# bitfrozen/rendering-algorithms-raytracer

Measured on AMD Instinct MI355X. Metric: Mray/s (primary+shadow) on Sponza 1920x1080, higher is better.
Workload: dtype f32; 1 GPU; sponza stand-in (~66k tris) 1920x1080 Blinn+PointLight; config=C3, width=1920, height=1080, spp=1, qbvh_nodes=9084, qbvh_leaves=18162, frames_in_flight=4, hw_queues=4, parallelism=single GPU, whole frame

## Files before the change

### rendering-algorithms-raytracer_amd/csrc/mrt_frame.hip

```cpp
#include "mrt_kernels.h"
#include "mrt_shader.h"

namespace mrt {

template <bool COUNT, bool FAST, bool POW, int WALK = 1>
__device__ __forceinline__ v3 shade1_hit(const RenderParams& P, const Trav& T, TravStats& st, const DRay& r, float ht,
                                         float ha, float hb, int prim, const uint16_t* rcpT, const uint16_t* rsqT,
                                         uint32_t& shadow_total) {
    const v3 rayD = mk(r.d[0], r.d[1], r.d[2]);
    const PrimShade ps = P.prims[prim];
    const uint32_t mi = ps.mat;
    const bool lambert = P.mats[mi].type == MRT_LAMBERT;
    const float4 A = P.verts[ps.v[0]], B = P.verts[ps.v[1]], C = P.verts[ps.v[2]];
    const v3 geoN = normalized(cross(mk(B.x - A.x, B.y - A.y, B.z - A.z), mk(C.x - A.x, C.y - A.y, C.z - A.z)), rsqT);
    const float c = 1.0f - ha - hb;
    const float4 n0 = P.normals[ps.n[0]], n1 = P.normals[ps.n[1]], n2 = P.normals[ps.n[2]];
    const v3 N = normalized(add(add(scale(mk(n0.x, n0.y, n0.z), c), scale(mk(n1.x, n1.y, n1.z), ha)),
                                scale(mk(n2.x, n2.y, n2.z), hb)), rsqT);
    const v3 from = mk(r.o[0] + ht * r.d[0], r.o[1] + ht * r.d[1], r.o[2] + ht * r.d[2]);
    v3 n = N, rVec = mk(0, 0, 0);
    if (!lambert) {
        const v3 viewDir = neg(rayD);
        float vDotN = dot(viewDir, N);
        const float vDotGeoN = dot(viewDir, geoN);
        const bool same = (vDotN * vDotGeoN) >= 0.0f;
        n = same ? N : geoN;
        vDotN = same ? vDotN : vDotGeoN;
        if (vDotN < 0.0f) { vDotN = -vDotN; n = neg(n); }
        rVec = add(rayD, scale(n, 2.0f * vDotN));
    }
    const DevLight& l = P.lights[0];
    v3 L = sub(mk(l.pos[0], l.pos[1], l.pos[2]), from);
    float nDotL = dot(n, L);
    float e = 0.f, spec = 0.f;
    if (nDotL > 0.0f) {
        float falloff = dot(L, L);
        const float distanceRecip = rsqrt_nr(falloff, rsqT);
        falloff = rcp_nr(falloff, rcpT);
        const float distance = rcp_nr(distanceRecip, rcpT);
        L = scale(L, distanceRecip);
        nDotL *= distanceRecip;
        float Aterm = (l.power * falloff) * (0.25f / 3.1415926f);
        float rdl = std_max(0.f, dot(rVec, L));
        asm volatile("" : "+v"(Aterm), "+v"(rdl), "+v"(nDotL));
        float attenuate = 1.0f;
        if (l.cast_shadows) {
            const DRay sr = make_ray(from, L);
            DHit sh{distance, 0.f, 0.f, -1};
            shadow_total++;
            if (traverse<true, COUNT, FAST, false, true, WALK == 2, WALK != 0>(T, sr, 0.001f, sh, st)) attenuate = 0.0f;
        }
        attenuate *= nDotL;
        spec = rdl * attenuate;
        e = Aterm * attenuate;
    }
    const DevMaterial& M = P.mats[mi];
    const v3 E = mk(e, e, e);
    const v3 kd = mk(M.kd[0], M.kd[1], M.kd[2]), ka = mk(M.ka[0], M.ka[1], M.ka[2]);
    v3 sh;
    if (lambert) {
        sh = add(add(mk(0, 0, 0), mul(E, kd)), ka);
    } else {
        const v3 ks = mk(M.ks[0], M.ks[1], M.ks[2]);
        const float pw = (!POW || M.spec_exp == 1.0f) ? spec : spec_pow(spec, M.spec_exp);
        const v3 Ls = add(mk(0, 0, 0), scale(scale(mul(E, ks), M.spec_amt), pw));
        const v3 Ld = add(add(mk(0, 0, 0), mul(E, kd)), ka);
        const v3 z = mk(0, 0, 0);
        sh = add(add(scale(add(add(Ld, Ls), z), 1.0f), scale(add(z, z), 1.0f)), mk(M.le[0], M.le[1], M.le[2]));
    }
    return add(mk(0, 0, 0), sh);
}

template <bool COUNT, bool FAST, int MINW, bool POW>
__global__ void __launch_bounds__(kWG, MINW) shade1_kernel(RenderParams P) {
    __shared__ uint16_t s_tab[2048];
    __shared__ int32_t s_stack[kLdsStack * kWG];
    load_tables(P.tables, s_tab, 1024);
    const uint64_t t0 = (COUNT || P.wave_log) ? wall_clock64() : 0;
    const uint16_t* rcpT = s_tab;
    const uint16_t* rsqT = P.tables + 2048;
    const int tid = threadIdx.x, lane = tid & 63, wave = tid >> 6;
    Trav T{P.nodes, P.fast_box != 0, P.scalar_nodes, P.leaves, rcpT, s_stack + tid, P.gstack + (blockIdx.x * kWG + tid), P.gstride};
    T.inst = P.insts;
    trav_alpha(T, P);
    TravStats st;
    uint32_t shadow_total = 0;
    TileSched ts(P, wave, lane);
    uint32_t ntiles = 0;
    for (int item = ts.first(); item >= 0; item = ts.next(item)) {
        if (P.wave_log && lane == 0 && ntiles < kLogTiles)
        {
            unsigned long long* r = P.wave_log + kLogWords * ((size_t)blockIdx.x * (kWG / 64) + wave);
            r[4 + ntiles] = ((unsigned long long)item << 40) | (wall_clock64() & ((1ull << 40) - 1));
            r[4 + kLogTiles + ntiles] = ts.deq_ticks;
        }
        ntiles++;
        int x, y;
        size_t slot;
        if (!item_pixel(P, item, lane, x, y, slot)) continue;
        const float4 hv = P.hits[slot];
        const int prim = __float_as_int(hv.w);
        v3 col = mk(P.bg[0], P.bg[1], P.bg[2]);
        if (prim >= 0) {
            const int f = item_frame(P, item);
            const EyeRay er = camera_ray(P.cam[f], P.seed + (uint32_t)f, x, y, rsqT);
            col = shade1_hit<COUNT, FAST, POW>(P, T, st, make_ray(er.o, er.d), hv.x, hv.y, hv.z, prim, rcpT, rsqT, shadow_total);
        }
        item_pixel(P, item, lane, x, y, slot);
        store_rgb(P, slot, col);
    }
    flush_stats<COUNT, false>(P, st, shadow_total, lane, t0, ntiles);
}

template <bool COUNT, bool FAST, int MINW, bool POW, int WALK = 1>
__global__ void __launch_bounds__(kWG, MINW) frame1_kernel(RenderParams P) {
    constexpr bool LN = WALK == 2;
    __shared__ uint16_t s_tab[2048];
    __shared__ int32_t s_stack[kLdsStack * kWG];
    __shared__ QNode s_top[LN ? kLdsNodes : 1];
    if (LN)
        for (int i = threadIdx.x; i < kLdsNodes * 32; i += kWG)
            reinterpret_cast<uint32_t*>(s_top)[i] = reinterpret_cast<const uint32_t*>(P.nodes)[i];
    load_tables(P.tables, s_tab, 1024);
    const uint64_t t0 = (COUNT || P.wave_log) ? wall_clock64() : 0;
    const uint16_t* rcpT = s_tab;
    const uint16_t* rsqT = P.tables + 2048;
    const int tid = threadIdx.x, lane = tid & 63, wave = __builtin_amdgcn_readfirstlane(tid >> 6);
    Trav T{P.nodes, P.fast_box != 0, P.scalar_nodes, P.leaves, rcpT, s_stack + tid, P.gstack + (blockIdx.x * kWG + tid), P.gstride};
    T.inst = P.insts;
    trav_alpha(T, P);
    if (LN) T.lnodes = s_top;
    TravStats st, ss;
    uint32_t nhits = 0, shadow_total = 0;
    unsigned long long wave_steps = 0, wave_steps_s = 0;
    TileSched ts(P, wave, lane);
    uint32_t ntiles = 0;
    for (int item = ts.first(); item >= 0; item = ts.next(item)) {
        const RenderParams& PA = reload_params();
        if (PA.wave_log && lane_id() == 0 && ntiles < kLogTiles) {
            unsigned long long* r = PA.wave_log + kLogWords * ((size_t)blockIdx.x * (kWG / 64) + wave);
            r[4 + ntiles] = ((unsigned long long)item << 40) | (wall_clock64() & ((1ull << 40) - 1));
            r[4 + kLogTiles + ntiles] = ts.deq_ticks;
        }
        ntiles++;
        int x, y;
        size_t slot;
        const uint32_t n0 = st.nodes, s0 = ss.nodes;
        if (item_pixel(PA, item, lane_id(), x, y, slot)) {
            const int f = item_frame(PA, item);
            const EyeRay er = camera_ray(PA.cam[f], PA.seed + (uint32_t)f, x, y, rsqT);
            const DRay r = make_ray(er.o, er.d);
            DHit h{1e12f, 0.f, 0.f, -1};
            const bool hit = traverse<false, COUNT, FAST, false, true, LN, WALK != 0, WALK == 3>(T, r, 0.001f, h, st);
            const RenderParams& PB = reload_params();
            v3 col = mk(PB.bg[0], PB.bg[1], PB.bg[2]);
            if (hit) {
                nhits++;
                col = shade1_hit<COUNT, FAST, POW, WALK>(PB, T, ss, r, h.t, h.a, h.b, h.prim, rcpT, rsqT, shadow_total);
            }
            const RenderParams& PC = reload_params();
            item_pixel(PC, item, lane_id(), x, y, slot);
            if (PC.hits) PC.hits[slot] = make_float4(h.t, h.a, h.b, __int_as_float(hit ? h.prim : -1));
            store_rgb(PC, slot, col);
        }
        if (COUNT) {
            uint32_t dmax = st.nodes - n0, smax = ss.nodes - s0;
            for (int off = 32; off > 0; off >>= 1) {
                dmax = max(dmax, (uint32_t)__shfl_xor(dmax, off));
                smax = max(smax, (uint32_t)__shfl_xor(smax, off));
            }
            wave_steps += dmax;
            wave_steps_s += smax;
        }
    }
    if (COUNT) {
        unsigned long long sv = ss.nodes;
        for (int off = 32; off > 0; off >>= 1) sv += __shfl_down(sv, off);
        if (lane_id() == 0) {
            atomicAdd(&P.ctr[CTR_WAVE_STEPS_P], wave_steps);
            atomicAdd(&P.ctr[CTR_WAVE_STEPS_S], wave_steps_s);
            atomicAdd(&P.ctr[CTR_NODES_S], sv);
        }
    }
    flush_stats<COUNT, true>(P, st, nhits, lane_id(), t0, ntiles, ss.nodes, wave);
    flush_stats<COUNT, false, false>(P, ss, shadow_total, lane_id(), t0, ntiles, 0, wave);
}

template <int W, bool POW>
static KernelFn shade1_fn(bool c, bool f) {
    return c ? (f ? shade1_kernel<true, true, W, POW> : shade1_kernel<true, false, W, POW>)
             : (f ? shade1_kernel<false, true, W, POW> : shade1_kernel<false, false, W, POW>);
}
template <int W, bool POW, int WALK>
static KernelFn frame1_fn(bool c, bool f) {
    return c ? (f ? frame1_kernel<true, true, W, POW, WALK> : frame1_kernel<true, false, W, POW, WALK>)
             : (f ? frame1_kernel<false, true, W, POW, WALK> : frame1_kernel<false, false, W, POW, WALK>);
}
template <int WALK>
static KernelFn pick_frame1_walk(int w, bool c, bool f, bool pow) {
    if (pow) return w == 1 ? frame1_fn<1, true, WALK>(c, f) : frame1_fn<6, true, WALK>(c, f);
    switch (w) {
        case 1: return frame1_fn<1, false, WALK>(c, f);
        case 5: return frame1_fn<5, false, WALK>(c, f);
        case 7: return frame1_fn<7, false, WALK>(c, f);
        case 8: return frame1_fn<8, false, WALK>(c, f);
        default: return frame1_fn<6, false, WALK>(c, f);
    }
}
KernelFn pick_frame1(int w, bool c, bool f, bool pow, int walk) {
    switch (walk) {
        case 0: return pick_frame1_walk<0>(w, c, f, pow);
        case 2: return pick_frame1_walk<2>(w, c, f, pow);
        case 3: return pick_frame1_walk<3>(w, c, f, pow);
        default: return pick_frame1_walk<1>(w, c, f, pow);
    }
}
KernelFn pick_shade1(bool c, bool f, bool pow) { return pow ? shade1_fn<5, true>(c, f) : shade1_fn<5, false>(c, f); }
}
```

### rendering-algorithms-raytracer_amd/csrc/mrt_kernels.h

```cpp
#pragma once
#include <hip/hip_runtime.h>

#include "../../include/mrt.h"
#include "mrt_math.h"
#include "mrt_texture.h"
#include "mrt_types.h"

namespace mrt {

static constexpr int kWG = 256;
static constexpr int kLdsStack = 16;
static constexpr int kGlobalStack = 240;
static constexpr int kTableWords = 4096;
static constexpr int kLdsNodes = 64;

struct DRay {
    float o[3], d[3], id[3];
    bool finite;
    float time;
};

__device__ __forceinline__ DRay make_ray(v3 o, v3 d) {
    DRay r;
    r.o[0] = o.x; r.o[1] = o.y; r.o[2] = o.z;
    r.d[0] = d.x; r.d[1] = d.y; r.d[2] = d.z;
#pragma unroll
    for (int k = 0; k < 3; k++) {
        float v = 1.0f / r.d[k];
        if (r.d[k] == 0.f) v = (v < -0.f) ? -1e12f : 1e12f;
        r.id[k] = v;
    }
    r.finite = __builtin_isfinite(r.o[0]) & __builtin_isfinite(r.o[1]) & __builtin_isfinite(r.o[2]) &
               __builtin_isfinite(r.id[0]) & __builtin_isfinite(r.id[1]) & __builtin_isfinite(r.id[2]);
    r.time = 0.f;
    return r;
}
__device__ __forceinline__ DRay make_ray(v3 o, v3 d, float time) {
    DRay r = make_ray(o, d);
    r.time = time;
    return r;
}

struct DHit {
    float t, a, b;
    int32_t prim;
    int32_t inst = -1;
};

struct Trav {
    const QNode* __restrict__ nodes;
    bool fast_box;
    int scalar_nodes;
    const DLeaf* __restrict__ leaves;
    const uint16_t* rcpT;
    int32_t* lds;
    int32_t* gstk;
    uint32_t gstride;
    const DevInstance* inst = nullptr;
    const PrimShade* aprims = nullptr;
    const uint4* apuv = nullptr;
    const float2* auv = nullptr;
    const DevMaterial* amats = nullptr;
    const DevTexture* atex = nullptr;
    const uint8_t* pflags = nullptr;
    const float4* verts = nullptr;
    const float4* verts2 = nullptr;
    bool near_first = false;
    const QNode* lnodes = nullptr;
};

struct TravStats {
    uint32_t nodes = 0, leaves = 0, uniform = 0;
    int max_sp = 0;
    bool overflow = false;
};

__device__ __forceinline__ bool stk_push(const Trav& c, int& sp, int32_t v) {
    if (sp < kLdsStack) c.lds[sp * kWG] = v;
    else if (sp < kLdsStack + kGlobalStack) c.gstk[(size_t)(sp - kLdsStack) * c.gstride] = v;
    else return false;
    sp++;
    return true;
}
__device__ __forceinline__ int32_t stk_pop(const Trav& c, int& sp) {
    --sp;
    return sp < kLdsStack ? c.lds[sp * kWG] : c.gstk[(size_t)(sp - kLdsStack) * c.gstride];
}

__device__ __forceinline__ int32_t sel4(const int4& v, int i) {
    const int32_t lo = (i & 1) ? v.y : v.x, hi = (i & 1) ? v.w : v.z;
    return (i & 2) ? hi : lo;
}

__device__ __forceinline__ bool tri_test(const float* __restrict__ T, const DRay& r, float tMin, float tBest,
                                         float& ot, float& oa, float& ob, const uint16_t* rcpT) {
    const float ax = T[0], ay = T[1], az = T[2], e0x = T[3], e0y = T[4], e0z = T[5], e1x = T[6], e1y = T[7], e1z = T[8];
    const float px = r.d[1] * e1z - r.d[2] * e1y;
    const float py = -1.0f * (r.d[0] * e1z - r.d[2] * e1x);
    const float pz = r.d[0] * e1y - r.d[1] * e1x;
    const float det = e0x * px + (e0y * py + e0z * pz);
    const float inv = rcp_nr(det, rcpT);
    const float tx = r.o[0] - ax, ty = r.o[1] - ay, tz = r.o[2] - az;
    const float a = inv * (tx * px + (ty * py + tz * pz));
    if (__ballot((a >= 0.0f) & (a <= 1.0f)) == 0) {
        ot = a; oa = a; ob = a;
        return false;
    }
    const float qx = ty * e0z - tz * e0y;
    const float qy = -1.0f * (tx * e0z - tz * e0x);
    const float qz = tx * e0y - ty * e0x;
    const float b = inv * (r.d[0] * qx + (r.d[1] * qy + r.d[2] * qz));
    const float t = inv * (e1x * qx + (e1y * qy + e1z * qz));
    ot = t; oa = a; ob = b;
    return (a >= 0.0f) & (b >= 0.0f) & ((a + b) <= 1.0f) & (t >= tMin) & (t < tBest);
}

__device__ __forceinline__ int box_test(const float4* bx, const DRay& r, float tMin, float tMax) {
    float4 mnx = bx[0], mny = bx[1], mnz = bx[2], mxx = bx[3], mxy = bx[4], mxz = bx[5];
    float lx[4] = {mnx.x, mnx.y, mnx.z, mnx.w}, ly[4] = {mny.x, mny.y, mny.z, mny.w}, lz[4] = {mnz.x, mnz.y, mnz.z, mnz.w};
    float hx[4] = {mxx.x, mxx.y, mxx.z, mxx.w}, hy[4] = {mxy.x, mxy.y, mxy.z, mxy.w}, hz[4] = {mxz.x, mxz.y, mxz.z, mxz.w};
    int m = 0;
#pragma unroll
    for (int i = 0; i < 4; i++) {
        float t0x = (lx[i] - r.o[0]) * r.id[0], t1x = (hx[i] - r.o[0]) * r.id[0];
        float t0y = (ly[i] - r.o[1]) * r.id[1], t1y = (hy[i] - r.o[1]) * r.id[1];
        float t0z = (lz[i] - r.o[2]) * r.id[2], t1z = (hz[i] - r.o[2]) * r.id[2];
        float t0 = sse_max(sse_min(t0x, t1x), sse_max(sse_min(t0y, t1y), sse_min(t0z, t1z)));
        float t1 = sse_min(sse_max(t0x, t1x), sse_min(sse_max(t0y, t1y), sse_max(t0z, t1z)));
        m |= (int)(sse_max(t0, tMin) <= sse_min(t1, tMax)) << i;
    }
    return m;
}

__device__ __forceinline__ int box_test_fast(const float4* bx, const DRay& r, float tMin, float tMax, int present = 15) {
    float4 mnx = bx[0], mny = bx[1], mnz = bx[2], mxx = bx[3], mxy = bx[4], mxz = bx[5];
    float lx[4] = {mnx.x, mnx.y, mnx.z, mnx.w}, ly[4] = {mny.x, mny.y, mny.z, mny.w}, lz[4] = {mnz.x, mnz.y, mnz.z, mnz.w};
    float hx[4] = {mxx.x, mxx.y, mxx.z, mxx.w}, hy[4] = {mxy.x, mxy.y, mxy.z, mxy.w}, hz[4] = {mxz.x, mxz.y, mxz.z, mxz.w};
    int m = 0;
#pragma unroll
    for (int i = 0; i < 4; i++) {
        if (i >= 2 && !((present >> i) & 1)) continue;
        float t0x = (lx[i] - r.o[0]) * r.id[0], t1x = (hx[i] - r.o[0]) * r.id[0];
        float t0y = (ly[i] - r.o[1]) * r.id[1], t1y = (hy[i] - r.o[1]) * r.id[1];
        float t0z = (lz[i] - r.o[2]) * r.id[2], t1z = (hz[i] - r.o[2]) * r.id[2];
        float t0 = __builtin_fmaxf(__builtin_fmaxf(__builtin_fminf(t0x, t1x), __builtin_fminf(t0y, t1y)),
                                   __builtin_fmaxf(__builtin_fminf(t0z, t1z), tMin));
        float t1 = __builtin_fminf(__builtin_fminf(__builtin_fmaxf(t0x, t1x), __builtin_fmaxf(t0y, t1y)),
                                   __builtin_fminf(__builtin_fmaxf(t0z, t1z), tMax));
        m |= (int)(t0 <= t1) << i;
    }
    return m;
}

template <int S>
__device__ __forceinline__ int box_test_oct(const float4* bx, const DRay& r, float tMin, float tMax, int present = 15) {
    const float4 nx = bx[(S & 1) ? 3 : 0], fx = bx[(S & 1) ? 0 : 3];
    const float4 ny = bx[(S & 2) ? 4 : 1], fy = bx[(S & 2) ? 1 : 4];
    const float4 nz = bx[(S & 4) ? 5 : 2], fz = bx[(S & 4) ? 2 : 5];
    const float lx[4] = {nx.x, nx.y, nx.z, nx.w}, ly[4] = {ny.x, ny.y, ny.z, ny.w}, lz[4] = {nz.x, nz.y, nz.z, nz.w};
    const float hx[4] = {fx.x, fx.y, fx.z, fx.w}, hy[4] = {fy.x, fy.y, fy.z, fy.w}, hz[4] = {fz.x, fz.y, fz.z, fz.w};
    int m = 0;
#pragma unroll
    for (int i = 0; i < 4; i++) {
        if (i >= 2 && !((present >> i) & 1)) continue;
        const float t0 = __builtin_fmaxf(__builtin_fmaxf((lx[i] - r.o[0]) * r.id[0], (ly[i] - r.o[1]) * r.id[1]),
                                         __builtin_fmaxf((lz[i] - r.o[2]) * r.id[2], tMin));
        const float t1 = __builtin_fminf(__builtin_fminf((hx[i] - r.o[0]) * r.id[0], (hy[i] - r.o[1]) * r.id[1]),
                                         __builtin_fminf((hz[i] - r.o[2]) * r.id[2], tMax));
        m |= (int)(t0 <= t1) << i;
    }
    return m;
}
__device__ __forceinline__ int box_test_sel(const float4* bx, const DRay& r, float tMin, float tMax, int s,
                                            int present = 15) {
    switch (s) {
        case 0: return box_test_oct<0>(bx, r, tMin, tMax, present);
        case 1: return box_test_oct<1>(bx, r, tMin, tMax, present);
        case 2: return box_test_oct<2>(bx, r, tMin, tMax, present);
        case 3: return box_test_oct<3>(bx, r, tMin, tMax, present);
        case 4: return box_test_oct<4>(bx, r, tMin, tMax, present);
        case 5: return box_test_oct<5>(bx, r, tMin, tMax, present);
        case 6: return box_test_oct<6>(bx, r, tMin, tMax, present);
        case 7: return box_test_oct<7>(bx, r, tMin, tMax, present);
        default: return box_test_fast(bx, r, tMin, tMax, present);
    }
}
__device__ __forceinline__ int wave_octant(const DRay& r) {
    const int oct = (int)(r.id[0] < 0.f) | (int)(r.id[1] < 0.f) << 1 | (int)(r.id[2] < 0.f) << 2;
    const int o0 = __builtin_amdgcn_readfirstlane(oct);
    return __ballot(oct != o0) == 0 ? o0 : 8;
}

__device__ __forceinline__ int box_test_fast_t(const float4* bx, const DRay& r, float tMin, float tMax, float (&tn)[4]) {
    float4 mnx = bx[0], mny = bx[1], mnz = bx[2], mxx = bx[3], mxy = bx[4], mxz = bx[5];
    float lx[4] = {mnx.x, mnx.y, mnx.z, mnx.w}, ly[4] = {mny.x, mny.y, mny.z, mny.w}, lz[4] = {mnz.x, mnz.y, mnz.z, mnz.w};
    float hx[4] = {mxx.x, mxx.y, mxx.z, mxx.w}, hy[4] = {mxy.x, mxy.y, mxy.z, mxy.w}, hz[4] = {mxz.x, mxz.y, mxz.z, mxz.w};
    int m = 0;
#pragma unroll
    for (int i = 0; i < 4; i++) {
        float t0x = (lx[i] - r.o[0]) * r.id[0], t1x = (hx[i] - r.o[0]) * r.id[0];
        float t0y = (ly[i] - r.o[1]) * r.id[1], t1y = (hy[i] - r.o[1]) * r.id[1];
        float t0z = (lz[i] - r.o[2]) * r.id[2], t1z = (hz[i] - r.o[2]) * r.id[2];
        float t0 = __builtin_fmaxf(__builtin_fmaxf(__builtin_fminf(t0x, t1x), __builtin_fminf(t0y, t1y)),
                                   __builtin_fmaxf(__builtin_fminf(t0z, t1z), tMin));
        float t1 = __builtin_fminf(__builtin_fminf(__builtin_fmaxf(t0x, t1x), __builtin_fmaxf(t0y, t1y)),
                                   __builtin_fminf(__builtin_fmaxf(t0z, t1z), tMax));
        tn[i] = t0;
        m |= (int)(t0 <= t1) << i;
    }
    return m;
}
__device__ __forceinline__ int nearest_slot(int bits, const float (&tn)[4]) {
    int best = 31 - __builtin_clz((unsigned)bits);
    float bt = tn[best];
#pragma unroll
    for (int i = 0; i < 4; i++)
        if (((bits >> i) & 1) && tn[i] < bt) { bt = tn[i]; best = i; }
    return best;
}

__host__ __device__ __forceinline__ int32_t leaf_child(uint32_t leaf, int count, bool proxy = false, bool check = false) {
    return ~(int32_t)((leaf << 4) | (check ? 8u : 0u) | (proxy ? 4u : 0u) | (uint32_t)(count - 1));
}

__host__ __device__ __forceinline__ uint32_t slot_kinds(const int32_t child[4]) {
    uint32_t k = 0;
    for (int i = 0; i < 4; i++) {
        const int32_t ch = child[i];
        if (ch >= 0) k |= 1u << i;
        else if (ch != kEmptySlot) k |= (1u << (4 + i)) | ((~(uint32_t)ch & 4u) ? 1u << (8 + i) : 0u);
    }
    return k;
}
__device__ __forceinline__ int node_kinds(const float4* q) { return reinterpret_cast<const int32_t*>(q)[28]; }
__device__ __forceinline__ int kinds_inner(int k) { return k & 15; }
__device__ __forceinline__ int kinds_leaf(int k) { return (k >> 4) & 15; }
__device__ __forceinline__ int kinds_proxy(int k) { return (k >> 8) & 15; }

__device__ __noinline__ bool mb_tri_test(const Trav& c, int32_t prim, const DRay& r, float tMin, float tBest, float& ot,
                                         float& oa, float& ob) {
    const PrimShade& ps = c.aprims[prim];
    const float time = r.time, _1_time = 1.f - time;
    const float4 a1 = c.verts[ps.v[0]], b1 = c.verts[ps.v[1]], c1 = c.verts[ps.v[2]];
    const float4 a2 = c.verts2[ps.v[0]], b2 = c.verts2[ps.v[1]], c2 = c.verts2[ps.v[2]];
    float T[9];
    T[0] = time * a2.x + _1_time * a1.x; T[1] = time * a2.y + _1_time * a1.y; T[2] = time * a2.z + _1_time * a1.z;
    T[3] = (time * b2.x + _1_time * b1.x) - T[0]; T[4] = (time * b2.y + _1_time * b1.y) - T[1];
    T[5] = (time * b2.z + _1_time * b1.z) - T[2];
    T[6] = (time * c2.x + _1_time * c1.x) - T[0]; T[7] = (time * c2.y + _1_time * c1.y) - T[1];
    T[8] = (time * c2.z + _1_time * c1.z) - T[2];
    return tri_test(T, r, tMin, tBest, ot, oa, ob, c.rcpT);
}

__device__ __noinline__
bool alpha_rejects(const Trav& c, uint32_t leaf, int k, float a, float b, int32_t aoff) {
    const int32_t prim = c.leaves[leaf].prim[k] + aoff;
    const int am = c.amats[c.aprims[prim].mat].maps[kMapAlpha];
    if (am < 0) return false;
    float u = a, v = b;
    if (c.apuv) {
        const uint4 t = c.apuv[prim];
        if (t.w) {
            const float cc = 1.0f - a - b;
            const float2 t0 = c.auv[t.x], t1 = c.auv[t.y], t2 = c.auv[t.z];
            u = t0.x * cc + t1.x * a + t2.x * b;
            v = t0.y * cc + t1.y * a + t2.y * b;
        }
    }
    const DevTexture& T = c.atex[am];
    return tex_lookup4(T.data, T.W, T.H, T.type, u, v).w < 0.5f;
}

__device__ __forceinline__ float dp4(const float* row, float x, float y, float z, float w) {
    const float p0 = row[0] * x, p1 = row[1] * y, p2 = row[2] * z, p3 = row[3] * w;
    return (p0 + p1) + (p2 + p3);
}

__device__ __forceinline__ DRay object_ray(const DevInstance& I, const DRay& r, const uint16_t* rcpT) {
    const float ox = r.o[0], oy = r.o[1], oz = r.o[2], dx = r.d[0], dy = r.d[1], dz = r.d[2];
    const float w = rcp_nr(dp4(I.inv + 12, ox, oy, oz, 1.0f), rcpT);
    const v3 o = mk(w * dp4(I.inv, ox, oy, oz, 1.0f), w * dp4(I.inv + 4, ox, oy, oz, 1.0f),
                    w * dp4(I.inv + 8, ox, oy, oz, 1.0f));
    const v3 d = mk(dp4(I.inv, dx, dy, dz, 0.0f), dp4(I.inv + 4, dx, dy, dz, 0.0f), dp4(I.inv + 8, dx, dy, dz, 0.0f));
    return make_ray(o, d, r.time);
}

__device__ __forceinline__ bool tri_test_lane(const Trav& c, uint32_t leaf, int k, const DRay& r, float tMin,
                                              float tBest, float& t, float& a, float& b) {
    int ok;
    const uint32_t key = (leaf << 2) | (uint32_t)k;
    const uint32_t k0 = __builtin_amdgcn_readfirstlane(key);
    if ((c.scalar_nodes & 2) && __ballot(key != k0) == 0) {
        typedef const __attribute__((address_space(4))) float cfloat;
        cfloat* q = (cfloat*)(const void*)(c.leaves[k0 >> 2].tri[k0 & 3]);
        float T[9];
#pragma unroll
        for (int i = 0; i < 9; i++) T[i] = q[i];
        ok = tri_test(T, r, tMin, tBest, t, a, b, c.rcpT) ? 1 : 0;
        asm volatile("; mrt: scalar triangle" : "+v"(ok));
    } else {
        ok = tri_test(c.leaves[leaf].tri[k], r, tMin, tBest, t, a, b, c.rcpT) ? 1 : 0;
        asm volatile("; mrt: vector triangle" : "+v"(ok));
    }
    return ok != 0;
}

template <bool ANY, bool COUNT, bool FAST, bool INST = false, bool BL = false, bool CHECK = true, bool LN = false,
          bool XONE = true, bool OL = false>
__device__ bool traverse_impl(const Trav& c, const DRay& r, float tMin, DHit& h, TravStats& st, int32_t root = 0,
                              int sp0 = 0, int32_t aoff = 0);

template <bool ANY, bool COUNT, bool FAST, bool CHECK = true>
__device__ __forceinline__ bool proxy_hit(const Trav& c, int inst, const DRay& r, float tMin, DHit& h,
                                          TravStats& st, int sp) {
    const DevInstance& I = c.inst[inst];
    const DRay ro = object_ray(I, r, c.rcpT);
    if (FAST && ro.finite)
        return traverse_impl<ANY, COUNT, true, false, true, CHECK, false, false>(c, ro, tMin, h, st, I.root, sp, I.shade_base);
    return traverse_impl<ANY, COUNT, false, false, true, CHECK, false, false>(c, ro, tMin, h, st, I.root, sp, I.shade_base);
}

template <bool ANY, bool COUNT, bool FAST, bool INST, bool BL, bool CHECK, bool LN, bool XONE, bool OL>
__device__ bool traverse_impl(const Trav& c, const DRay& r, float tMin, DHit& h, TravStats& st, int32_t root,
                              int sp0, int32_t aoff) {
    int sp = sp0;
    int32_t cur = root;
    bool hit = false;
    const int soct = (FAST && !(ANY && c.near_first) && (c.scalar_nodes & 4)) ? wave_octant(r) : 8;
    while (true) {
        const int32_t peek = c.lds[__builtin_elementwise_min((uint32_t)(sp - 1), (uint32_t)(kLdsStack - 1)) * kWG];
        int m, kinds;
        int4 ch;
        const int32_t c0 = __builtin_amdgcn_readfirstlane(cur);
        float tn[4] = {0.f, 0.f, 0.f, 0.f};
        if (LN && FAST && c0 < kLdsNodes && __ballot(cur != c0) == 0) {
            const QNode& nd = c.lnodes[c0];
            ch = make_int4(nd.child[0], nd.child[1], nd.child[2], nd.child[3]);
            kinds = (int)nd.pad[0];
            float4 bx[6];
#pragma unroll
            for (int k = 0; k < 6; k++) bx[k] = make_float4(nd.box[4 * k], nd.box[4 * k + 1], nd.box[4 * k + 2], nd.box[4 * k + 3]);
            m = (ANY && c.near_first) ? box_test_fast_t(bx, r, tMin, h.t, tn) : box_test_sel(bx, r, tMin, h.t, soct);
            asm volatile("; mrt: lds node" : "+v"(m));
        } else if (FAST && (c.scalar_nodes & 1) && __ballot(cur != c0) == 0) {
            typedef const __attribute__((address_space(4))) float cfloat;
            typedef const __attribute__((address_space(4))) int32_t cint;
            cfloat* q = (cfloat*)(const void*)(c.nodes + c0);
            cint* qc = (cint*)(q + 24);
            ch = make_int4(qc[0], qc[1], qc[2], qc[3]);
            kinds = qc[4];
            float4 bx[6];
#pragma unroll
            for (int k = 0; k < 6; k++) bx[k] = make_float4(q[4 * k], q[4 * k + 1], q[4 * k + 2], q[4 * k + 3]);
            const int present = __builtin_amdgcn_readfirstlane((kinds | (kinds >> 4)) & 15);
            m = (ANY && c.near_first) ? box_test_fast_t(bx, r, tMin, h.t, tn)
                                      : box_test_sel(bx, r, tMin, h.t, soct, present);
            asm volatile("; mrt: scalar node" : "+v"(m));
        } else {
            const float4* q = reinterpret_cast<const float4*>(c.nodes + cur);
            ch = reinterpret_cast<const int4*>(q)[6];
            kinds = node_kinds(q);
            m = FAST ? ((ANY && c.near_first) ? box_test_fast_t(q, r, tMin, h.t, tn) : box_test_sel(q, r, tMin, h.t, soct))
                     : box_test(q, r, tMin, h.t);
            asm volatile("; mrt: vector node" : "+v"(m));
        }
        if (COUNT) {
            st.nodes++;
            if (__ballot(cur != c0) == 0) st.uniform++;
        }
        const int inner = m & kinds_inner(kinds);
        int lm = m & kinds_leaf(kinds);
        bool have_next = false;
        int32_t nxt = 0;
        if (inner) {
            const int top = (FAST && ANY && c.near_first) ? nearest_slot(inner, tn) : 31 - __builtin_clz((unsigned)inner);
            const int rest = inner ^ (1 << top);
            bool ovf = false;
            if (rest) {
                if (sp + 4 <= kLdsStack) {
                    c.lds[sp * kWG] = ch.x; sp += rest & 1;
                    c.lds[sp * kWG] = ch.y; sp += (rest >> 1) & 1;
                    c.lds[sp * kWG] = ch.z; sp += (rest >> 2) & 1;
                    c.lds[sp * kWG] = ch.w; sp += (rest >> 3) & 1;
                } else {
                    bool pushed = true;
#pragma unroll
                    for (int i = 0; i < 4; i++)
                        if ((rest >> i) & 1) pushed = pushed && stk_push(c, sp, sel4(ch, i));
                    if (!pushed) {
                        st.overflow = true;
                        if (!XONE) return hit;
                        sp = sp0;
                        ovf = true;
                    }
                }
                if (COUNT && sp > st.max_sp) st.max_sp = sp;
            }
            nxt = sel4(ch, top);
            have_next = !ovf;
        }
        if (lm) {
            uint32_t leaf = 0;
            int k = 0, cnt = 0;
            bool check = false;
            while (true) {
                if (k == cnt) {
                    if (!lm) break;
                    const int s = __builtin_ctz((unsigned)lm);
                    lm &= lm - 1;
                    const uint32_t v = ~(uint32_t)sel4(ch, s);
                    leaf = v >> 4;
                    cnt = (int)(v & 3u) + 1;
                    k = 0;
                    check = CHECK && (INST || BL) && (v & 8u);
                    if (COUNT) st.leaves++;
                    if (INST && (v & 4u)) {
                        for (int j = 0; j < cnt; j++) {
                            const int32_t pm = c.leaves[leaf].prim[j];
                            if (pm > -2) continue;
                            DHit hi{h.t, 0.f, 0.f, -1};
                            const bool ph = proxy_hit<ANY, COUNT, FAST, CHECK>(c, -2 - pm, r, tMin, hi, st, sp);
                            if (st.overflow) return hit;
                            if (ph) {
                                if (ANY) return true;
                                h.t = hi.t; h.a = hi.a; h.b = hi.b; h.prim = hi.prim; h.inst = -2 - pm;
                                hit = true;
                            }
                        }
                    }
                }
                float t, a, b;
                bool ok;
                if (CHECK && (INST || BL) && check) {
                    const int32_t pm = c.leaves[leaf].prim[k];
                    ok = (!BL && pm >= 0 && c.pflags && (c.pflags[pm] & 1u))
                             ? mb_tri_test(c, pm, r, tMin, h.t, t, a, b)
                             : tri_test(c.leaves[leaf].tri[k], r, tMin, h.t, t, a, b, c.rcpT);
                    ok = ok && !alpha_rejects(c, leaf, k, a, b, aoff);
                } else {
                    ok = tri_test_lane(c, leaf, k, r, tMin, h.t, t, a, b);
                }
                if (ok) {
                    if (ANY) return true;
                    h.t = t; h.a = a; h.b = b; h.prim = (int32_t)((leaf << 2) | (uint32_t)k);
                    if (INST) h.inst = -1;
                    hit = true;
                }
                k++;
            }
        }
        if (OL) {
            int32_t g = peek;
            const uint32_t lds_left = sp0 < kLdsStack ? (uint32_t)(kLdsStack - sp0) : 0u;
            if (!have_next && (uint32_t)(sp - 1 - sp0) >= lds_left) {
                if (sp == sp0) break;
                g = c.gstk[(size_t)(sp - 1 - kLdsStack) * c.gstride];
            }
            cur = have_next ? nxt : g;
            sp -= have_next ? 0 : 1;
        } else if (have_next) {
            cur = nxt;
        } else {
            if (sp == sp0) break;
            if (sp <= kLdsStack) { cur = peek; sp--; }
            else cur = stk_pop(c, sp);
        }
    }
    return hit;
}

template <bool COUNT, bool FAST>
__device__ __forceinline__ bool anyhit_step(const Trav& c, const DRay& r, float tMin, float tMax, int32_t& cur,
                                            int& sp, bool& hit, TravStats& st) {
    int m, kinds;
    int4 ch;
    const int32_t c0 = __builtin_amdgcn_readfirstlane(cur);
    float tn[4] = {0.f, 0.f, 0.f, 0.f};
    if (FAST && (c.scalar_nodes & 1) && __ballot(cur != c0) == 0) {
        typedef const __attribute__((address_space(4))) float cfloat;
        typedef const __attribute__((address_space(4))) int32_t cint;
        cfloat* q = (cfloat*)(const void*)(c.nodes + c0);
        cint* qc = (cint*)(q + 24);
        ch = make_int4(qc[0], qc[1], qc[2], qc[3]);
        kinds = qc[4];
        float4 bx[6];
#pragma unroll
        for (int k = 0; k < 6; k++) bx[k] = make_float4(q[4 * k], q[4 * k + 1], q[4 * k + 2], q[4 * k + 3]);
        m = c.near_first ? box_test_fast_t(bx, r, tMin, tMax, tn) : box_test_fast(bx, r, tMin, tMax);
        asm volatile("; mrt: scalar node" : "+v"(m));
    } else {
        const float4* q = reinterpret_cast<const float4*>(c.nodes + cur);
        ch = reinterpret_cast<const int4*>(q)[6];
        kinds = node_kinds(q);
        m = FAST ? (c.near_first ? box_test_fast_t(q, r, tMin, tMax, tn) : box_test_fast(q, r, tMin, tMax))
                 : box_test(q, r, tMin, tMax);
        asm volatile("; mrt: vector node" : "+v"(m));
    }
    if (COUNT) st.nodes++;
    const int inner = m & kinds_inner(kinds);
    int lm = m & kinds_leaf(kinds);
    bool have_next = false;
    int32_t nxt = 0;
    if (inner) {
        const int top = (FAST && c.near_first) ? nearest_slot(inner, tn) : 31 - __builtin_clz((unsigned)inner);
        const int rest = inner ^ (1 << top);
        if (rest) {
            if (sp + 4 <= kLdsStack) {
                c.lds[sp * kWG] = ch.x; sp += rest & 1;
                c.lds[sp * kWG] = ch.y; sp += (rest >> 1) & 1;
                c.lds[sp * kWG] = ch.z; sp += (rest >> 2) & 1;
                c.lds[sp * kWG] = ch.w; sp += (rest >> 3) & 1;
            } else {
#pragma unroll
                for (int i = 0; i < 4; i++)
                    if ((rest >> i) & 1)
                        if (!stk_push(c, sp, sel4(ch, i))) { st.overflow = true; return true; }
            }
            if (COUNT && sp > st.max_sp) st.max_sp = sp;
        }
        nxt = sel4(ch, top);
        have_next = true;
    }
    if (lm) {
        uint32_t leaf = 0;
        int k = 0, cnt = 0;
        while (true) {
            if (k == cnt) {
                if (!lm) break;
                const int s = __builtin_ctz((unsigned)lm);
                lm &= lm - 1;
                const uint32_t v = ~(uint32_t)sel4(ch, s);
                leaf = v >> 4;
                cnt = (int)(v & 3u) + 1;
                k = 0;
                if (COUNT) st.leaves++;
            }
            float t, a, b;
            if (tri_test(c.leaves[leaf].tri[k], r, tMin, tMax, t, a, b, c.rcpT)) { hit = true; return true; }
            k++;
        }
    }
    if (have_next) { cur = nxt; return false; }
    if (sp == 0) return true;
    cur = stk_pop(c, sp);
    return false;
}

struct AnyState {
    DRay q;
    int32_t cur;
    int sp;
    int32_t aoff;
};
template <bool COUNT, bool FAST, bool CHECK>
__device__ __forceinline__ bool anyhit_step_inst(const Trav& c, float tMin, float tMax, AnyState& s,
                                                 const float4* ray_o, const float4* ray_d, uint32_t e, bool& hit,
                                                 TravStats& st) {
    if (s.cur == -1) {
        const float4 o = ray_o[e], d = ray_d[e];
        s.q = make_ray(mk(o.x, o.y, o.z), mk(d.x, d.y, d.z), d.w);
        s.aoff = -1;
        if (s.sp == 0) return true;
        s.cur = stk_pop(c, s.sp);
    }
    if (s.cur <= -2) {
        const int i = -2 - s.cur;
        if (!stk_push(c, s.sp, -1)) { st.overflow = true; return true; }
        s.q = object_ray(c.inst[i], s.q, c.rcpT);
        s.cur = c.inst[i].root;
        s.aoff = c.inst[i].shade_base;
    }
    const DRay& q = s.q;
    const float4* qn = reinterpret_cast<const float4*>(c.nodes + s.cur);
    const int4 ch = reinterpret_cast<const int4*>(qn)[6];
    const int kinds = node_kinds(qn);
    float tn[4] = {0.f, 0.f, 0.f, 0.f};
    const bool fast = FAST && q.finite;
    const int m = fast ? (c.near_first ? box_test_fast_t(qn, q, tMin, tMax, tn) : box_test_fast(qn, q, tMin, tMax))
                       : box_test(qn, q, tMin, tMax);
    if (COUNT) st.nodes++;
    const int inner = m & kinds_inner(kinds);
    int lm = m & kinds_leaf(kinds);
    const bool proxies = (lm & kinds_proxy(kinds)) != 0;
    bool have_next = false;
    int32_t nxt = 0;
    if (inner) {
        const int top = (fast && c.near_first) ? nearest_slot(inner, tn) : 31 - __builtin_clz((unsigned)inner);
        const int rest = proxies ? inner : inner ^ (1 << top);
        if (rest) {
            if (s.sp + 4 <= kLdsStack) {
                c.lds[s.sp * kWG] = ch.x; s.sp += rest & 1;
                c.lds[s.sp * kWG] = ch.y; s.sp += (rest >> 1) & 1;
                c.lds[s.sp * kWG] = ch.z; s.sp += (rest >> 2) & 1;
                c.lds[s.sp * kWG] = ch.w; s.sp += (rest >> 3) & 1;
            } else {
#pragma unroll
                for (int i = 0; i < 4; i++)
                    if ((rest >> i) & 1)
                        if (!stk_push(c, s.sp, sel4(ch, i))) { st.overflow = true; return true; }
            }
            if (COUNT && s.sp > st.max_sp) st.max_sp = s.sp;
        }
        nxt = sel4(ch, top);
        have_next = !proxies;
    }
    while (lm) {
        const int sl = __builtin_ctz((unsigned)lm);
        lm &= lm - 1;
        const uint32_t v = ~(uint32_t)sel4(ch, sl);
        const uint32_t leaf = v >> 4;
        const int cnt = (int)(v & 3u) + 1;
        if (COUNT) st.leaves++;
        for (int k = 0; k < cnt; k++) {
            if (v & 4u) {
                const int32_t pm = c.leaves[leaf].prim[k];
                if (pm <= -2) {
                    if (!stk_push(c, s.sp, pm)) { st.overflow = true; return true; }
                    continue;
                }
            }
            float t, a, b;
            bool ok;
            if (CHECK && (v & 8u)) {
                const int32_t pm = c.leaves[leaf].prim[k];
                ok = (s.aoff < 0 && pm >= 0 && c.pflags && (c.pflags[pm] & 1u))
                         ? mb_tri_test(c, pm, q, tMin, tMax, t, a, b)
                         : tri_test(c.leaves[leaf].tri[k], q, tMin, tMax, t, a, b, c.rcpT);
                ok = ok && !alpha_rejects(c, leaf, k, a, b, s.aoff < 0 ? 0 : s.aoff);
            } else {
                ok = tri_test(c.leaves[leaf].tri[k], q, tMin, tMax, t, a, b, c.rcpT);
            }
            if (ok) { hit = true; return true; }
        }
    }
    if (have_next) { s.cur = nxt; return false; }
    if (s.sp == 0) return true;
    s.cur = stk_pop(c, s.sp);
    return false;
}

template <bool ANY, bool COUNT, bool FAST = false, bool INST = false, bool CHECK = true, bool LN = false,
          bool XONE = false, bool OL = false>
__device__ __forceinline__ bool traverse(const Trav& c, const DRay& r, float tMin, DHit& h, TravStats& st) {
    const bool hit = (FAST && r.finite) ? traverse_impl<ANY, COUNT, true, INST, false, CHECK, LN, XONE, OL>(c, r, tMin, h, st)
                                        : traverse_impl<ANY, COUNT, false, INST, false, CHECK, false, XONE, OL>(c, r, tMin, h, st);
    if (!ANY && hit) {
        h.prim = c.leaves[(uint32_t)h.prim >> 2].prim[h.prim & 3];
        if (INST && h.inst >= 0) h.prim += c.inst[h.inst].hit_base;
    }
    return hit;
}

}
```

Baseline: 11750 Mray/s.

## Load octant-ordered node box rows into scalar registers for uniform-octant waves

```diff
diff --git a/rendering-algorithms-raytracer_amd/csrc/mrt_frame.hip b/rendering-algorithms-raytracer_amd/csrc/mrt_frame.hip
--- a/rendering-algorithms-raytracer_amd/csrc/mrt_frame.hip
+++ b/rendering-algorithms-raytracer_amd/csrc/mrt_frame.hip
@@ -48,7 +48,7 @@
             const DRay sr = make_ray(from, L);
             DHit sh{distance, 0.f, 0.f, -1};
             shadow_total++;
-            if (traverse<true, COUNT, FAST, false, true, WALK == 2, WALK != 0>(T, sr, 0.001f, sh, st)) attenuate = 0.0f;
+            if (traverse<true, COUNT, FAST, false, true, WALK == 2, WALK != 0, false, true>(T, sr, 0.001f, sh, st)) attenuate = 0.0f;
         }
         attenuate *= nDotL;
         spec = rdl * attenuate;
@@ -151,7 +151,7 @@
             const EyeRay er = camera_ray(PA.cam[f], PA.seed + (uint32_t)f, x, y, rsqT);
             const DRay r = make_ray(er.o, er.d);
             DHit h{1e12f, 0.f, 0.f, -1};
-            const bool hit = traverse<false, COUNT, FAST, false, true, LN, WALK != 0, WALK == 3>(T, r, 0.001f, h, st);
+            const bool hit = traverse<false, COUNT, FAST, false, true, LN, WALK != 0, WALK == 3, true>(T, r, 0.001f, h, st);
             const RenderParams& PB = reload_params();
             v3 col = mk(PB.bg[0], PB.bg[1], PB.bg[2]);
             if (hit) {
diff --git a/rendering-algorithms-raytracer_amd/csrc/mrt_kernels.h b/rendering-algorithms-raytracer_amd/csrc/mrt_kernels.h
--- a/rendering-algorithms-raytracer_amd/csrc/mrt_kernels.h
+++ b/rendering-algorithms-raytracer_amd/csrc/mrt_kernels.h
@@ -171,6 +171,25 @@
     }
     return m;
 }
+struct OctRows {
+    uint32_t nx, ny, nz, fx, fy, fz;
+};
+__device__ __forceinline__ OctRows oct_rows(int s) {
+    OctRows o;
+    o.nx = (s & 1) ? 12u : 0u; o.fx = 12u - o.nx;
+    o.ny = (s & 2) ? 16u : 4u; o.fy = 20u - o.ny;
+    o.nz = (s & 4) ? 20u : 8u; o.fz = 28u - o.nz;
+    return o;
+}
+__device__ __forceinline__ void pin_rows(float4 (&bx)[6]) {
+    typedef float f4 __attribute__((ext_vector_type(4)));
+    f4 v[6];
+#pragma unroll
+    for (int k = 0; k < 6; k++) v[k] = f4{bx[k].x, bx[k].y, bx[k].z, bx[k].w};
+    asm volatile("" : "+s"(v[0]), "+s"(v[1]), "+s"(v[2]), "+s"(v[3]), "+s"(v[4]), "+s"(v[5]));
+#pragma unroll
+    for (int k = 0; k < 6; k++) bx[k] = make_float4(v[k].x, v[k].y, v[k].z, v[k].w);
+}
 __device__ __forceinline__ int box_test_sel(const float4* bx, const DRay& r, float tMin, float tMax, int s,
                                             int present = 15) {
     switch (s) {
@@ -289,8 +308,8 @@
                                               float tBest, float& t, float& a, float& b) {
     int ok;
     const uint32_t key = (leaf << 2) | (uint32_t)k;
-    const uint32_t k0 = __builtin_amdgcn_readfirstlane(key);
-    if ((c.scalar_nodes & 2) && __ballot(key != k0) == 0) {
+    const uint32_t k0 = __builtin_amdgcn_readfirstlane(key) ^ ((c.scalar_nodes & 2) ? 0u : 0x80000000u);
+    if (__ballot(key != k0) == 0) {
         typedef const __attribute__((address_space(4))) float cfloat;
         cfloat* q = (cfloat*)(const void*)(c.leaves[k0 >> 2].tri[k0 & 3]);
         float T[9];
@@ -306,7 +325,7 @@
 }
 
 template <bool ANY, bool COUNT, bool FAST, bool INST = false, bool BL = false, bool CHECK = true, bool LN = false,
-          bool XONE = true, bool OL = false>
+          bool XONE = true, bool OL = false, bool OROWS = false>
 __device__ bool traverse_impl(const Trav& c, const DRay& r, float tMin, DHit& h, TravStats& st, int32_t root = 0,
                               int sp0 = 0, int32_t aoff = 0);
 
@@ -320,13 +339,14 @@
     return traverse_impl<ANY, COUNT, false, false, true, CHECK, false, false>(c, ro, tMin, h, st, I.root, sp, I.shade_base);
 }
 
-template <bool ANY, bool COUNT, bool FAST, bool INST, bool BL, bool CHECK, bool LN, bool XONE, bool OL>
+template <bool ANY, bool COUNT, bool FAST, bool INST, bool BL, bool CHECK, bool LN, bool XONE, bool OL, bool OROWS>
 __device__ bool traverse_impl(const Trav& c, const DRay& r, float tMin, DHit& h, TravStats& st, int32_t root,
                               int sp0, int32_t aoff) {
     int sp = sp0;
     int32_t cur = root;
-    bool hit = false;
     const int soct = (FAST && !(ANY && c.near_first) && (c.scalar_nodes & 4)) ? wave_octant(r) : 8;
+    const bool orows = OROWS && FAST && (c.scalar_nodes & 1) && soct < 8;
+    const OctRows rows = oct_rows(soct);
     while (true) {
         const int32_t peek = c.lds[__builtin_elementwise_min((uint32_t)(sp - 1), (uint32_t)(kLdsStack - 1)) * kWG];
         int m, kinds;
@@ -342,6 +362,24 @@
             for (int k = 0; k < 6; k++) bx[k] = make_float4(nd.box[4 * k], nd.box[4 * k + 1], nd.box[4 * k + 2], nd.box[4 * k + 3]);
             m = (ANY && c.near_first) ? box_test_fast_t(bx, r, tMin, h.t, tn) : box_test_sel(bx, r, tMin, h.t, soct);
             asm volatile("; mrt: lds node" : "+v"(m));
+        } else if (orows && __ballot(cur != c0) == 0) {
+            typedef const __attribute__((address_space(4))) float cfloat;
+            typedef const __attribute__((address_space(4))) int32_t cint;
+            cfloat* q = (cfloat*)(const void*)(c.nodes + c0);
+            cint* qc = (cint*)(q + 24);
+            ch = make_int4(qc[0], qc[1], qc[2], qc[3]);
+            kinds = qc[4];
+            const uint32_t ro[6] = {rows.nx, rows.ny, rows.nz, rows.fx, rows.fy, rows.fz};
+            float4 bx[6];
+#pragma unroll
+            for (int k = 0; k < 6; k++) {
+                cfloat* qr = q + ro[k];
+                bx[k] = make_float4(qr[0], qr[1], qr[2], qr[3]);
+            }
+            pin_rows(bx);
+            const int present = __builtin_amdgcn_readfirstlane((kinds | (kinds >> 4)) & 15);
+            m = box_test_oct<0>(bx, r, tMin, h.t, present);
+            asm volatile("; mrt: scalar node" : "+v"(m));
         } else if (FAST && (c.scalar_nodes & 1) && __ballot(cur != c0) == 0) {
             typedef const __attribute__((address_space(4))) float cfloat;
             typedef const __attribute__((address_space(4))) int32_t cint;
@@ -352,10 +390,12 @@
             float4 bx[6];
 #pragma unroll
             for (int k = 0; k < 6; k++) bx[k] = make_float4(q[4 * k], q[4 * k + 1], q[4 * k + 2], q[4 * k + 3]);
+            if (OROWS) pin_rows(bx);
             const int present = __builtin_amdgcn_readfirstlane((kinds | (kinds >> 4)) & 15);
             m = (ANY && c.near_first) ? box_test_fast_t(bx, r, tMin, h.t, tn)
+                : OROWS               ? box_test_fast(bx, r, tMin, h.t, present)
                                       : box_test_sel(bx, r, tMin, h.t, soct, present);
-            asm volatile("; mrt: scalar node" : "+v"(m));
+            asm volatile("; mrt: scalar node, any octant" : "+v"(m));
         } else {
             const float4* q = reinterpret_cast<const float4*>(c.nodes + cur);
             ch = reinterpret_cast<const int4*>(q)[6];
@@ -370,12 +410,11 @@
         }
         const int inner = m & kinds_inner(kinds);
         int lm = m & kinds_leaf(kinds);
-        bool have_next = false;
-        int32_t nxt = 0;
+        int32_t nxt = -1;
         if (inner) {
             const int top = (FAST && ANY && c.near_first) ? nearest_slot(inner, tn) : 31 - __builtin_clz((unsigned)inner);
             const int rest = inner ^ (1 << top);
-            bool ovf = false;
+            nxt = sel4(ch, top);
             if (rest) {
                 if (sp + 4 <= kLdsStack) {
                     c.lds[sp * kWG] = ch.x; sp += rest & 1;
@@ -389,16 +428,15 @@
                         if ((rest >> i) & 1) pushed = pushed && stk_push(c, sp, sel4(ch, i));
                     if (!pushed) {
                         st.overflow = true;
-                        if (!XONE) return hit;
+                        if (!XONE) return !ANY && h.prim >= 0;
                         sp = sp0;
-                        ovf = true;
+                        nxt = -1;
                     }
                 }
                 if (COUNT && sp > st.max_sp) st.max_sp = sp;
             }
-            nxt = sel4(ch, top);
-            have_next = !ovf;
-        }
+        }
+        const bool have_next = nxt >= 0;
         if (lm) {
             uint32_t leaf = 0;
             int k = 0, cnt = 0;
@@ -420,11 +458,10 @@
                             if (pm > -2) continue;
                             DHit hi{h.t, 0.f, 0.f, -1};
                             const bool ph = proxy_hit<ANY, COUNT, FAST, CHECK>(c, -2 - pm, r, tMin, hi, st, sp);
-                            if (st.overflow) return hit;
+                            if (st.overflow) return !ANY && h.prim >= 0;
                             if (ph) {
                                 if (ANY) return true;
                                 h.t = hi.t; h.a = hi.a; h.b = hi.b; h.prim = hi.prim; h.inst = -2 - pm;
-                                hit = true;
                             }
                         }
                     }
@@ -444,7 +481,6 @@
                     if (ANY) return true;
                     h.t = t; h.a = a; h.b = b; h.prim = (int32_t)((leaf << 2) | (uint32_t)k);
                     if (INST) h.inst = -1;
-                    hit = true;
                 }
                 k++;
             }
@@ -466,7 +502,7 @@
             else cur = stk_pop(c, sp);
         }
     }
-    return hit;
+    return !ANY && h.prim >= 0;
 }
 
 template <bool COUNT, bool FAST>
@@ -640,9 +676,9 @@
 }
 
 template <bool ANY, bool COUNT, bool FAST = false, bool INST = false, bool CHECK = true, bool LN = false,
-          bool XONE = false, bool OL = false>
+          bool XONE = false, bool OL = false, bool OROWS = false>
 __device__ __forceinline__ bool traverse(const Trav& c, const DRay& r, float tMin, DHit& h, TravStats& st) {
-    const bool hit = (FAST && r.finite) ? traverse_impl<ANY, COUNT, true, INST, false, CHECK, LN, XONE, OL>(c, r, tMin, h, st)
+    const bool hit = (FAST && r.finite) ? traverse_impl<ANY, COUNT, true, INST, false, CHECK, LN, XONE, OL, OROWS>(c, r, tMin, h, st)
                                         : traverse_impl<ANY, COUNT, false, INST, false, CHECK, false, XONE, OL>(c, r, tMin, h, st);
     if (!ANY && hit) {
         h.prim = c.leaves[(uint32_t)h.prim >> 2].prim[h.prim & 3];
```

Result: faster. 12850 Mray/s (median of 6 runs) (+9.4%).
